# instadeepai/FrameDiPT

Measured on AMD Instinct MI355X. Metric: residue*diffusion-steps/sec, higher is better.
Workload: dtype fp16

## Files before the change

framedipt_amd/csrc/frames.hip:

```cpp
#include "common.hpp"
#include "kernels.hpp"
#include "philox.hpp"

#pragma clang fp contract(off)

__device__ __forceinline__ void d_quat_to_rot(const float* q, float* R) {
  const float a = q[0], b = q[1], c = q[2], d = q[3];
  R[0] = a * a + b * b - c * c - d * d; R[1] = 2 * b * c - 2 * a * d; R[2] = 2 * b * d + 2 * a * c;
  R[3] = 2 * b * c + 2 * a * d; R[4] = a * a - b * b + c * c - d * d; R[5] = 2 * c * d - 2 * a * b;
  R[6] = 2 * b * d - 2 * a * c; R[7] = 2 * c * d + 2 * a * b; R[8] = a * a - b * b - c * c + d * d;
}
__device__ __forceinline__ void d_quat_mul(const float* p, const float* q, float* o) {
  o[0] = p[0] * q[0] - p[1] * q[1] - p[2] * q[2] - p[3] * q[3];
  o[1] = p[0] * q[1] + p[1] * q[0] + p[2] * q[3] - p[3] * q[2];
  o[2] = p[0] * q[2] - p[1] * q[3] + p[2] * q[0] + p[3] * q[1];
  o[3] = p[0] * q[3] + p[1] * q[2] - p[2] * q[1] + p[3] * q[0];
}
__device__ __forceinline__ void d_quat_mul_vec(const float* q, const float* v, float* o) {
  o[0] = -q[1] * v[0] - q[2] * v[1] - q[3] * v[2];
  o[1] = q[0] * v[0] + q[2] * v[2] - q[3] * v[1];
  o[2] = q[0] * v[1] - q[1] * v[2] + q[3] * v[0];
  o[3] = q[0] * v[2] + q[1] * v[1] - q[2] * v[0];
}
__device__ __forceinline__ void d_invert_quat(const float* q, float* o) {
// ... 71 lines not shown
  for (int i = 0; i < 3; ++i)
    for (int j = 0; j < 3; ++j) Ro[i * 3 + j] = R1[i * 3] * R2[j] + R1[i * 3 + 1] * R2[3 + j] + R1[i * 3 + 2] * R2[6 + j];
  float tmp[3];
  d_rot_vec(R1, t2, tmp);
  to[0] = tmp[0] + t1[0]; to[1] = tmp[1] + t1[1]; to[2] = tmp[2] + t1[2];
}

__device__ __forceinline__ void d_backbone_residue(long r, const float* Rb, const float* tbv, const float* __restrict__ psi,
                                                   const int32_t* __restrict__ aatype, const BackboneTables* __restrict__ tb,
                                                   float* __restrict__ atom37, float* __restrict__ atom14) {
  int aa = aatype ? aatype[r] : 0;
  if (aa == 20) aa = 0;
  const float s = psi[r * 2], co = psi[r * 2 + 1];
  float FR[8][9], FT[8][3];
  for (int g = 0; g < 8; ++g) {
    const float* d44 = tb->default_frames + (aa * 8 + g) * 16;
    float Rd[9], td[3], Ra[9];
    for (int i = 0; i < 3; ++i) {
      for (int j = 0; j < 3; ++j) Rd[i * 3 + j] = d44[i * 4 + j];
      td[i] = d44[i * 4 + 3];
    }
    const float a0 = g == 0 ? 0.f : s, a1 = g == 0 ? 1.f : co;
    Ra[0] = 1; Ra[1] = 0; Ra[2] = 0; Ra[3] = 0; Ra[4] = a1; Ra[5] = -a0; Ra[6] = 0; Ra[7] = a0; Ra[8] = a1;
    const float z3[3] = {0.f, 0.f, 0.f};
    d_compose(Rd, td, Ra, z3, FR[g], FT[g]);
  }
  for (int g = 5; g < 8; ++g) {
    float Rn[9], tn[3];
    d_compose(FR[g - 1], FT[g - 1], FR[g], FT[g], Rn, tn);
    for (int c = 0; c < 9; ++c) FR[g][c] = Rn[c];
    for (int c = 0; c < 3; ++c) FT[g][c] = tn[c];
  }
  float pos[14][3];
  for (int at = 0; at < 14; ++at) {
    const int g = tb->group_idx[aa * 14 + at];
    float Rg[9], tg[3], p[3];
    d_compose(Rb, tbv, FR[g], FT[g], Rg, tg);
    d_rot_vec(Rg, tb->ideal_pos + (aa * 14 + at) * 3, p);
    const float mk = tb->atom_mask[aa * 14 + at];
    for (int c = 0; c < 3; ++c) pos[at][c] = (p[c] + tg[c]) * mk;
  }
  if (atom14)
    for (int at = 0; at < 14; ++at)
      for (int c = 0; c < 3; ++c) fd_st(atom14 + (r * 14 + at) * 3 + c, pos[at][c]);
  if (atom37) {
    for (int c = 0; c < 37 * 3; ++c) atom37[r * 111 + c] = 0.f;
    const int map[5] = {0, 1, 2, 4, 3};
    for (int at = 0; at < 5; ++at)
      for (int c = 0; c < 3; ++c) fd_st(atom37 + r * 111 + at * 3 + c, pos[map[at]][c]);
  }
}

__device__ __forceinline__ void d_backbone_atom(int at, int aa, float s, float co, const float* Rb, const float* tbv,
                                                const BackboneTables* __restrict__ tb, float* p3) {
  const int g = tb->group_idx[aa * 14 + at];
  auto frame = [&](int gg, float* R, float* T) {
    const float* d44 = tb->default_frames + (aa * 8 + gg) * 16;
    float Rd[9], td[3], Ra[9];
    for (int i = 0; i < 3; ++i) {
      for (int j = 0; j < 3; ++j) Rd[i * 3 + j] = d44[i * 4 + j];
      td[i] = d44[i * 4 + 3];
    }
    const float a0 = gg == 0 ? 0.f : s, a1 = gg == 0 ? 1.f : co;
    Ra[0] = 1; Ra[1] = 0; Ra[2] = 0; Ra[3] = 0; Ra[4] = a1; Ra[5] = -a0; Ra[6] = 0; Ra[7] = a0; Ra[8] = a1;
    const float z3[3] = {0.f, 0.f, 0.f};
    d_compose(Rd, td, Ra, z3, R, T);
  };
  float FRg[9], FTg[3];
  frame(g < 5 ? g : 4, FRg, FTg);
  for (int gg = 5; gg <= g; ++gg) {
    float Rc[9], Tc[3], Rn[9], Tn[3];
    frame(gg, Rc, Tc);
    d_compose(FRg, FTg, Rc, Tc, Rn, Tn);
    for (int c = 0; c < 9; ++c) FRg[c] = Rn[c];
    for (int c = 0; c < 3; ++c) FTg[c] = Tn[c];
  }
  float Rg[9], tg[3], p[3];
  d_compose(Rb, tbv, FRg, FTg, Rg, tg);
  d_rot_vec(Rg, tb->ideal_pos + (aa * 14 + at) * 3, p);
  const float mk = tb->atom_mask[aa * 14 + at];
  for (int c = 0; c < 3; ++c) p3[c] = (p[c] + tg[c]) * mk;
}

struct ReverseArgs {
  int B, N;
  const float* rigids_t;
  const double* rot_score;
  const float* trans_score;
  const float* diffuse_mask;
  const double *z_rot, *z_trans;
  double t, dt, noise_scale;
  int center, diffuse_rot, diffuse_trans;
  double so3_min_sigma, so3_max_sigma, r3_min_b, r3_max_b, cs;
  float* rigids_out;
  float* out_rot;
  int rpb;
  const float* psi;
  const int32_t* aatype;
  const BackboneTables* tables;
  float* atom37;
  const float* pred_rigids;
  const float* traj_fixed;
  float* trans_traj;
  int32_t* cursor = nullptr;
  const double* t_table = nullptr;
};

struct NoiseKeys { const uint64_t* keys; int step; };
template <bool GEN, typename... G>
__global__ __launch_bounds__(FD_THREADS) void reverse_step_kernel(ReverseArgs a, G... gs) {
  static_assert(sizeof...(G) == (GEN ? 1 : 0), "noise keys ride along with GEN only");
  __shared__ double red[4][FD_THREADS / 64];
  __shared__ double com[4];
  const int b = blockIdx.y, tid = threadIdx.x, lane = tid & 63, wave = tid >> 6;
  const int N = a.N;
  uint64_t key = 0;
  int step = 0;
  if constexpr (GEN) {
    const NoiseKeys g = (gs, ...);
    key = g.keys[b];
    step = a.cursor ? a.cursor[0] : g.step;
  }
  if (a.cursor) {
    const long s = a.cursor[0], R = (long)a.B * N;
    a.rigids_t += s * R * 7;
    a.rigids_out += (s + 1) * R * 7;
    if (!GEN) {
      a.z_rot += s * R * 3;
      a.z_trans += s * R * 3;
    }
    a.t = a.t_table[s];
    if (a.atom37) a.atom37 += s * R * 111;
    if (a.trans_traj) a.trans_traj += s * R * 3;
  }
  const double emax = exp(a.so3_max_sigma), emin = exp(a.so3_min_sigma);
  const double sig = log(a.t * emax + (1 - a.t) * emin);
  const double g_rot = sqrt(2 * (emax - emin) * sig / exp(sig));
  const double bt = a.r3_min_b + a.t * (a.r3_max_b - a.r3_min_b);
  const double g_tr = sqrt(bt);
  const double sdt = sqrt(a.dt);
  double sx = 0, sy = 0, sz = 0, sm = 0;
  for (int i = tid; i < N; i += FD_THREADS) {
    const long r = (long)b * N + i;
    const double m = a.diffuse_mask ? (double)a.diffuse_mask[r] : 1.0;
    double x1[3], zt[3] = {0.0, 0.0, 0.0};
    if (GEN && a.diffuse_trans) fd_noise3(key, (uint32_t)i, (uint32_t)step, FD_NOISE_REV_TRANS, zt);
    for (int c = 0; c < 3; ++c) {
      const double x = (double)a.rigids_t[r * 7 + 4 + c] * a.cs;
      const double f = -0.5 * bt * x;
      const double z = a.noise_scale * (GEN ? zt[c] : a.z_trans[r * 3 + c]);
      double pert = (f - g_tr * g_tr * (double)a.trans_score[r * 3 + c]) * a.dt + g_tr * sdt * z;
      pert *= m;
      x1[c] = x - pert;
    }
    sx += x1[0]; sy += x1[1]; sz += x1[2]; sm += m;
  }
  sx = wave_sum_d(sx); sy = wave_sum_d(sy); sz = wave_sum_d(sz); sm = wave_sum_d(sm);
  if (lane == 0) { red[0][wave] = sx; red[1][wave] = sy; red[2][wave] = sz; red[3][wave] = sm; }
  __syncthreads();
  if (tid < 4) {
    double s = 0;
    for (int w = 0; w < FD_THREADS / 64; ++w) s += red[tid][w];
    com[tid] = s;
  }
  __syncthreads();
  const double cx = a.center ? com[0] / com[3] : 0.0, cy = a.center ? com[1] / com[3] : 0.0,
               cz = a.center ? com[2] / com[3] : 0.0;
  const int i_end = (int)(blockIdx.x + 1) * a.rpb < N ? (int)(blockIdx.x + 1) * a.rpb : N;
  for (int i = blockIdx.x * a.rpb + tid; i < i_end; i += FD_THREADS) {
    const long r = (long)b * N + i;
    const bool has_mask = a.diffuse_mask != nullptr;
    const double m = has_mask ? (double)a.diffuse_mask[r] : 1.0;
    double tr_out[3], zt[3] = {0.0, 0.0, 0.0}, zr[3] = {0.0, 0.0, 0.0};
    if (GEN && a.diffuse_trans) fd_noise3(key, (uint32_t)i, (uint32_t)step, FD_NOISE_REV_TRANS, zt);
    for (int c = 0; c < 3; ++c) {
      const double xt = (double)a.rigids_t[r * 7 + 4 + c];
      double x1 = xt;
      if (a.diffuse_trans) {
        const double x = xt * a.cs;
        const double f = -0.5 * bt * x;
        const double z = a.noise_scale * (GEN ? zt[c] : a.z_trans[r * 3 + c]);
        double pert = (f - g_tr * g_tr * (double)a.trans_score[r * 3 + c]) * a.dt + g_tr * sdt * z;
        pert *= m;
        x1 = x - pert;
        x1 -= (c == 0 ? cx : (c == 1 ? cy : cz));
        x1 = x1 / a.cs;
      }
      tr_out[c] = has_mask ? (m * x1 + (1 - m) * xt) : x1;
    }
    float R32[9];
    d_quat_to_rot(a.rigids_t + r * 7, R32);
    double Rt[9], Ro[9];
    for (int c = 0; c < 9; ++c) Rt[c] = (double)R32[c];
    double pert[3];
    if (GEN && a.diffuse_rot) fd_noise3(key, (uint32_t)i, (uint32_t)step, FD_NOISE_REV_ROT, zr);
    for (int c = 0; c < 3; ++c)
      pert[c] = g_rot * g_rot * a.rot_score[r * 3 + c] * a.dt + g_rot * sdt * (a.noise_scale * (GEN ? zr[c] : a.z_rot[r * 3 + c]));
    if (!has_mask || m == 1.0 || m == 0.0) {
      double q0[4];
      d_markley(Rt, q0);
      if (a.diffuse_rot && m != 0.0) {
        double Re[9], Rp[9], Rc[9], q1[4];
        d_quat_matrix(q0, Re);
        d_so3_exp(pert, Rp);
        for (int ii = 0; ii < 3; ++ii)
          for (int jj = 0; jj < 3; ++jj)
            Rc[ii * 3 + jj] = Re[ii * 3] * Rp[jj] + Re[ii * 3 + 1] * Rp[3 + jj] + Re[ii * 3 + 2] * Rp[6 + jj];
        d_markley(Rc, q1);
        d_quat_matrix(q1, Ro);
      } else {
        d_quat_matrix(q0, Ro);
      }
    } else {
    double rv[3];
    d_so3_log(Rt, rv);
    double rv1[3] = {rv[0], rv[1], rv[2]};
    if (a.diffuse_rot) {
      double Rp[9], Rc[9];
      double Re[9];
      d_so3_exp(rv, Re);
      d_so3_exp(pert, Rp);
      for (int ii = 0; ii < 3; ++ii)
        for (int jj = 0; jj < 3; ++jj)
          Rc[ii * 3 + jj] = Re[ii * 3] * Rp[jj] + Re[ii * 3 + 1] * Rp[3 + jj] + Re[ii * 3 + 2] * Rp[6 + jj];
      d_so3_log(Rc, rv1);
    }
    if (has_mask)
      for (int c = 0; c < 3; ++c) rv1[c] = m * rv1[c] + (1 - m) * rv[c];
    d_so3_exp(rv1, Ro);
    }
    float Rf[9];
    for (int c = 0; c < 9; ++c) Rf[c] = (float)Ro[c];
    if (a.out_rot)
      for (int c = 0; c < 9; ++c) fd_st(a.out_rot + r * 9 + c, Rf[c]);
    double Rd[9], q[4];
    for (int c = 0; c < 9; ++c) Rd[c] = (double)Rf[c];
    d_markley(Rd, q);
    if (q[3] < 0) { q[0] = -q[0]; q[1] = -q[1]; q[2] = -q[2]; q[3] = -q[3]; }
    float* o = a.rigids_out + r * 7;
    fd_st(o, (float)q[3]); fd_st(o + 1, (float)q[0]); fd_st(o + 2, (float)q[1]); fd_st(o + 3, (float)q[2]);
    fd_st(o + 4, (float)tr_out[0]); fd_st(o + 5, (float)tr_out[1]); fd_st(o + 6, (float)tr_out[2]);
    if (a.atom37) {
      const float tf[3] = {o[4], o[5], o[6]};
      d_backbone_residue(r, Rf, tf, a.psi, a.aatype, a.tables, a.atom37, nullptr);
    }
    if (a.trans_traj) {
      const float dm = a.diffuse_mask ? a.diffuse_mask[r] : 1.f, fm = a.traj_fixed[r];
      for (int c = 0; c < 3; ++c) fd_st(a.trans_traj + r * 3 + c, dm * a.pred_rigids[r * 7 + 4 + c] + fm * o[4 + c]);
    }
  }
  if (a.cursor) {
    __syncthreads();
// ... 520 lines not shown
}

#define FD_EW_EXPORT(name, X, Y, O, O2)                                                        \
  if (n <= 0) return FDIPT_OK;                                                                 \
  if (!(X) || !(O)) return FDIPT_EINVAL;                                                       \
  hipLaunchKernelGGL(name##_k, dim3(cdiv(n, 256)), dim3(256), 0, (hipStream_t)s, n, X, Y, O, O2); \
  FD_CHECK_LAUNCH();                                                                           \
  return FDIPT_OK;

extern "C" {
int fdipt_quat_to_rot(int n, const float* quat, float* rot, fdipt_stream_t s) { FD_EW_EXPORT(quat_to_rot, quat, nullptr, rot, nullptr) }
int fdipt_rot_to_quat(int n, const float* rot, float* quat, fdipt_stream_t s) { FD_EW_EXPORT(rot_to_quat, rot, nullptr, quat, nullptr) }
int fdipt_quat_multiply(int n, const float* q1, const float* q2, float* out, fdipt_stream_t s) { FD_EW_EXPORT(quat_multiply, q1, q2, out, nullptr) }
int fdipt_quat_multiply_by_vec(int n, const float* q, const float* v, float* out, fdipt_stream_t s) { FD_EW_EXPORT(quat_multiply_by_vec, q, v, out, nullptr) }
int fdipt_invert_quat(int n, const float* q, float* out, fdipt_stream_t s) { FD_EW_EXPORT(invert_quat, q, nullptr, out, nullptr) }
int fdipt_rigid_apply(int n, const float* t7, const float* pts, float* out, fdipt_stream_t s) { FD_EW_EXPORT(rigid_apply, t7, pts, out, nullptr) }
int fdipt_rigid_invert_apply(int n, const float* t7, const float* pts, float* out, fdipt_stream_t s) { FD_EW_EXPORT(rigid_invert_apply, t7, pts, out, nullptr) }
int fdipt_rigid_compose(int n, const float* a, const float* b, float* out_rot, float* out_trans, fdipt_stream_t s) { FD_EW_EXPORT(rigid_compose, a, b, out_rot, out_trans) }
int fdipt_rigid_invert(int n, const float* t7, float* out_rot, float* out_trans, fdipt_stream_t s) { FD_EW_EXPORT(rigid_invert, t7, nullptr, out_rot, out_trans) }
int fdipt_quat_to_rotvec(int n, const float* q, float* rotvec, fdipt_stream_t s) { FD_EW_EXPORT(quat_to_rotvec, q, nullptr, rotvec, nullptr) }

int fdipt_rigid_compose_q_update(int n, const float* t7, const float* upd6, const float* mask, float* out_t7,
                                 fdipt_stream_t s) {
  if (n <= 0) return FDIPT_OK;
  if (!t7 || !upd6 || !out_t7) return FDIPT_EINVAL;
  hipLaunchKernelGGL(cqu_t7_k, dim3(cdiv(n, 256)), dim3(256), 0, (hipStream_t)s, n, t7, upd6, mask, out_t7);
  FD_CHECK_LAUNCH();
  return FDIPT_OK;
}
int fdipt_rigid_from_3_points(int n, const float* p_neg_x_axis, const float* origin, const float* p_xy_plane, float eps, float* rot,
                              fdipt_stream_t s) {
  if (n <= 0) return FDIPT_OK;
  if (!p_neg_x_axis || !origin || !p_xy_plane || !rot) return FDIPT_EINVAL;
  hipLaunchKernelGGL(from_3_points_k, dim3(cdiv(n, 256)), dim3(256), 0, (hipStream_t)s, n, p_neg_x_axis, origin, p_xy_plane, eps, rot);
  FD_CHECK_LAUNCH();
  return FDIPT_OK;
}
int fdipt_so3_exp_geomstats(int n, const double* rotvec, double* rot, fdipt_stream_t s) {
  if (n <= 0) return FDIPT_OK;
  if (!rotvec || !rot) return FDIPT_EINVAL;
  hipLaunchKernelGGL(gs_exp_k, dim3(cdiv(n, 256)), dim3(256), 0, (hipStream_t)s, n, rotvec, rot);
  FD_CHECK_LAUNCH();
  return FDIPT_OK;
}
int fdipt_so3_log_geomstats(int n, const double* rot, double* rotvec, fdipt_stream_t s) {
  if (n <= 0) return FDIPT_OK;
  if (!rotvec || !rot) return FDIPT_EINVAL;
  hipLaunchKernelGGL(gs_log_k, dim3(cdiv(n, 256)), dim3(256), 0, (hipStream_t)s, n, rot, rotvec);
  FD_CHECK_LAUNCH();
  return FDIPT_OK;
}
int fdipt_so3_omega(int n, const double* rot, double eps, double* angle, fdipt_stream_t s) {
  if (n <= 0) return FDIPT_OK;
  if (!angle || !rot) return FDIPT_EINVAL;
  hipLaunchKernelGGL(gs_omega_k, dim3(cdiv(n, 256)), dim3(256), 0, (hipStream_t)s, n, rot, eps, angle);
  FD_CHECK_LAUNCH();
  return FDIPT_OK;
}
int fdipt_so3_exp(int n, const double* rotvec, double* rot, fdipt_stream_t s) {
  if (n <= 0) return FDIPT_OK;
  if (!rotvec || !rot) return FDIPT_EINVAL;
  hipLaunchKernelGGL(so3_exp_k, dim3(cdiv(n, 256)), dim3(256), 0, (hipStream_t)s, n, rotvec, rot);
  FD_CHECK_LAUNCH();
  return FDIPT_OK;
}
int fdipt_so3_log(int n, const double* rot, double* rotvec, fdipt_stream_t s) {
  if (n <= 0) return FDIPT_OK;
  if (!rot || !rotvec) return FDIPT_EINVAL;
  hipLaunchKernelGGL(so3_log_k, dim3(cdiv(n, 256)), dim3(256), 0, (hipStream_t)s, n, rot, rotvec);
  FD_CHECK_LAUNCH();
  return FDIPT_OK;
}

int fdipt_se3_reverse_step_atoms(int B, int N, const float* rigids_t, const double* rot_score, const float* trans_score,
                                 const float* diffuse_mask, const double* z_rot, const double* z_trans, double t, double dt,
                                 double noise_scale, int center, int diffuse_rot, int diffuse_trans, double so3_min_sigma,
                                 double so3_max_sigma, double r3_min_b, double r3_max_b, double coordinate_scaling,
                                 float* rigids_out, float* out_rot, const float* psi, const int32_t* aatype,
                                 const void* tables, float* atom37, fdipt_stream_t stream) {
  if (B <= 0 || N <= 0) return FDIPT_OK;
  if (!rigids_t || !rot_score || !trans_score || !z_rot || !z_trans || !rigids_out || !(t >= 0 && t <= 1))
    return FDIPT_EINVAL;
  if (atom37 && (!psi || !tables || rigids_out == rigids_t)) return FDIPT_EINVAL;
  const int rpb = rigids_out == rigids_t ? N : 64;
  ReverseArgs a = {B, N, rigids_t, rot_score, trans_score, diffuse_mask, z_rot, z_trans, t, dt, noise_scale, center,
                   diffuse_rot, diffuse_trans, so3_min_sigma, so3_max_sigma, r3_min_b, r3_max_b, coordinate_scaling,
                   rigids_out, out_rot, rpb, psi, aatype, (const BackboneTables*)tables, atom37, nullptr, nullptr, nullptr};
  hipLaunchKernelGGL(reverse_step_kernel<false>, dim3(cdiv(N, rpb), B), dim3(FD_THREADS), 0, (hipStream_t)stream, a);
  FD_CHECK_LAUNCH();
  return FDIPT_OK;
}
int fdipt_se3_reverse_step_traj(int B, int N, const float* rigids_t, const double* rot_score, const float* trans_score,
                                const float* diffuse_mask, const double* z_rot, const double* z_trans, double t, double dt,
                                double noise_scale, int center, int diffuse_rot, int diffuse_trans, double so3_min_sigma,
                                double so3_max_sigma, double r3_min_b, double r3_max_b, double coordinate_scaling,
                                float* rigids_out, float* out_rot, const float* psi, const int32_t* aatype,
                                const void* tables, float* atom37, const float* pred_rigids, const float* traj_fixed_mask,
                                float* trans_traj, fdipt_stream_t stream) {
  if (B <= 0 || N <= 0) return FDIPT_OK;
  if (!rigids_t || !rot_score || !trans_score || !z_rot || !z_trans || !rigids_out || !(t >= 0 && t <= 1))
    return FDIPT_EINVAL;
  if (atom37 && (!psi || !tables || rigids_out == rigids_t)) return FDIPT_EINVAL;
  if (trans_traj && (!pred_rigids || !traj_fixed_mask)) return FDIPT_EINVAL;
  const int rpb = rigids_out == rigids_t ? N : 64;
  ReverseArgs a = {B, N, rigids_t, rot_score, trans_score, diffuse_mask, z_rot, z_trans, t, dt, noise_scale, center,
                   diffuse_rot, diffuse_trans, so3_min_sigma, so3_max_sigma, r3_min_b, r3_max_b, coordinate_scaling,
                   rigids_out, out_rot, rpb, psi, aatype, (const BackboneTables*)tables, atom37, pred_rigids, traj_fixed_mask, trans_traj};
  hipLaunchKernelGGL(reverse_step_kernel<false>, dim3(cdiv(N, rpb), B), dim3(FD_THREADS), 0, (hipStream_t)stream, a);
  FD_CHECK_LAUNCH();
  return FDIPT_OK;
}
int fdipt_se3_reverse_step_indexed(const FdiptReverseIndexed* x, fdipt_stream_t stream) {
  if (!x) return FDIPT_EINVAL;
  if (x->B <= 0 || x->N <= 0) return FDIPT_OK;
  if (!x->rigid_traj || !x->rot_score || !x->trans_score || !x->z_rot || !x->z_trans || !x->t_table || !x->step_cursor) return FDIPT_EINVAL;
  if (x->prot_traj && (!x->psi || !x->bb_tables)) return FDIPT_EINVAL;
  if (x->trans_traj && (!x->pred_rigids || !x->traj_fixed_mask)) return FDIPT_EINVAL;
  ReverseArgs a = {x->B, x->N, x->rigid_traj, x->rot_score, x->trans_score, x->diffuse_mask, x->z_rot, x->z_trans, 0.0, x->dt,
                   x->noise_scale, x->center, x->diffuse_rot, x->diffuse_trans, x->so3_min_sigma, x->so3_max_sigma, x->r3_min_b,
                   x->r3_max_b, x->coordinate_scaling, x->rigid_traj, nullptr, 64, x->psi, x->aatype,
                   (const BackboneTables*)x->bb_tables, x->prot_traj, x->pred_rigids, x->traj_fixed_mask, x->trans_traj,
                   x->step_cursor, x->t_table};
  hipLaunchKernelGGL(reverse_step_kernel<false>, dim3(cdiv(x->N, 64), x->B), dim3(FD_THREADS), 0, (hipStream_t)stream, a);
  FD_CHECK_LAUNCH();
  return FDIPT_OK;
}
int fdipt_se3_reverse_step_traj_gen(int B, int N, const float* rigids_t, const double* rot_score, const float* trans_score,
                                    const float* diffuse_mask, const uint64_t* noise_keys, int step, double t, double dt,
                                    double noise_scale, int center, int diffuse_rot, int diffuse_trans, double so3_min_sigma,
                                    double so3_max_sigma, double r3_min_b, double r3_max_b, double coordinate_scaling,
                                    float* rigids_out, float* out_rot, const float* psi, const int32_t* aatype,
                                    const void* tables, float* atom37, const float* pred_rigids, const float* traj_fixed_mask,
                                    float* trans_traj, fdipt_stream_t stream) {
  if (B <= 0 || N <= 0) return FDIPT_OK;
  if (!rigids_t || !rot_score || !trans_score || !noise_keys || step < 0 || !rigids_out || !(t >= 0 && t <= 1))
    return FDIPT_EINVAL;
  if (atom37 && (!psi || !tables || rigids_out == rigids_t)) return FDIPT_EINVAL;
  if (trans_traj && (!pred_rigids || !traj_fixed_mask)) return FDIPT_EINVAL;
  const int rpb = rigids_out == rigids_t ? N : 64;
  ReverseArgs a = {B, N, rigids_t, rot_score, trans_score, diffuse_mask, nullptr, nullptr, t, dt, noise_scale, center,
                   diffuse_rot, diffuse_trans, so3_min_sigma, so3_max_sigma, r3_min_b, r3_max_b, coordinate_scaling,
                   rigids_out, out_rot, rpb, psi, aatype, (const BackboneTables*)tables, atom37, pred_rigids, traj_fixed_mask, trans_traj};
  hipLaunchKernelGGL((reverse_step_kernel<true, NoiseKeys>), dim3(cdiv(N, rpb), B), dim3(FD_THREADS), 0, (hipStream_t)stream, a, NoiseKeys{noise_keys, step});
  FD_CHECK_LAUNCH();
  return FDIPT_OK;
}
int fdipt_se3_reverse_step_indexed_gen(const FdiptReverseIndexed* x, const uint64_t* noise_keys, fdipt_stream_t stream) {
  if (!x) return FDIPT_EINVAL;
  if (x->B <= 0 || x->N <= 0) return FDIPT_OK;
  if (!x->rigid_traj || !x->rot_score || !x->trans_score || x->z_rot || x->z_trans || !noise_keys || !x->t_table || !x->step_cursor)
    return FDIPT_EINVAL;
  if (x->prot_traj && (!x->psi || !x->bb_tables)) return FDIPT_EINVAL;
  if (x->trans_traj && (!x->pred_rigids || !x->traj_fixed_mask)) return FDIPT_EINVAL;
  ReverseArgs a = {x->B, x->N, x->rigid_traj, x->rot_score, x->trans_score, x->diffuse_mask, nullptr, nullptr, 0.0, x->dt,
                   x->noise_scale, x->center, x->diffuse_rot, x->diffuse_trans, x->so3_min_sigma, x->so3_max_sigma, x->r3_min_b,
                   x->r3_max_b, x->coordinate_scaling, x->rigid_traj, nullptr, 64, x->psi, x->aatype,
                   (const BackboneTables*)x->bb_tables, x->prot_traj, x->pred_rigids, x->traj_fixed_mask, x->trans_traj,
                   x->step_cursor, x->t_table};
  hipLaunchKernelGGL((reverse_step_kernel<true, NoiseKeys>), dim3(cdiv(x->N, 64), x->B), dim3(FD_THREADS), 0, (hipStream_t)stream, a, NoiseKeys{noise_keys, 0});
  FD_CHECK_LAUNCH();
  return FDIPT_OK;
}
int fdipt_noise_fill(int B, int N, const uint64_t* noise_keys, int purpose, int k_begin, int n_steps, double* out, fdipt_stream_t stream) {
  if (B <= 0 || N <= 0 || n_steps <= 0) return FDIPT_OK;
  if (!noise_keys || !out || purpose < 0 || purpose >= (int)FD_NOISE_PURPOSES || k_begin < 0) return FDIPT_EINVAL;
  const long n = (long)n_steps * B * N;
  hipLaunchKernelGGL(noise_fill_kernel, dim3(cdiv(n, FD_THREADS)), dim3(FD_THREADS), 0, (hipStream_t)stream, B, N, noise_keys,
                     (uint32_t)purpose, k_begin, n, out);
  FD_CHECK_LAUNCH();
  return FDIPT_OK;
}
int fdipt_se3_reverse_step(int B, int N, const float* rigids_t, const double* rot_score, const float* trans_score,
                           const float* diffuse_mask, const double* z_rot, const double* z_trans, double t, double dt,
                           double noise_scale, int center, int diffuse_rot, int diffuse_trans, double so3_min_sigma,
                           double so3_max_sigma, double r3_min_b, double r3_max_b, double coordinate_scaling,
                           float* rigids_out, float* out_rot, fdipt_stream_t stream) {
  return fdipt_se3_reverse_step_atoms(B, N, rigids_t, rot_score, trans_score, diffuse_mask, z_rot, z_trans, t, dt, noise_scale,
                                      center, diffuse_rot, diffuse_trans, so3_min_sigma, so3_max_sigma, r3_min_b, r3_max_b,
                                      coordinate_scaling, rigids_out, out_rot, nullptr, nullptr, nullptr, nullptr, stream);
}

int fdipt_igso3_rot_score(int B, int N, const float* quats_t, const float* quats_0, const double* sigma,
                          const float* res_mask, double* score, fdipt_stream_t s) {
  if (B <= 0 || N <= 0) return FDIPT_OK;
  if (!quats_t || !quats_0 || !sigma || !score) return FDIPT_EINVAL;
  return fd_rot_score(B, N, quats_t, 4, quats_0, 4, sigma, res_mask, score, (hipStream_t)s);
}
int fdipt_igso3_rot_score_cached(int B, int N, const float* quats_t, const float* quats_0, const double* score_table,
                                 const double* omega_edges, int n_omega, const float* res_mask, double* score, fdipt_stream_t s) {
  if (B <= 0 || N <= 0) return FDIPT_OK;
  if (!quats_t || !quats_0 || !score_table || !omega_edges || n_omega < 2 || !score) return FDIPT_EINVAL;
  ScoreTail x = {};
  x.score_table = score_table; x.omega_edges = omega_edges; x.n_omega = n_omega;
  hipLaunchKernelGGL(rot_score_kernel, dim3(cdiv((long)B * N, FD_THREADS / RS_LANES)), dim3(FD_THREADS), 0, (hipStream_t)s, B, N, quats_t, 4,
                     quats_0, 4, score_table, res_mask, score, x);
  FD_CHECK_LAUNCH();
  return FDIPT_OK;
}
int fdipt_r3_trans_score(int B, int N, const float* trans_t, const float* trans_0, const float* t, float min_b,
                         float max_b, float coordinate_scaling, const float* res_mask, float* score, fdipt_stream_t s) {
  if (B <= 0 || N <= 0) return FDIPT_OK;
  if (!trans_t || !trans_0 || !t || !score) return FDIPT_EINVAL;
  return fd_trans_score(B, N, trans_t, 3, trans_0, 3, t, min_b, max_b, coordinate_scaling, res_mask, score, (hipStream_t)s);
}
int fdipt_backbone_atoms(int n, const float* t7, const float* rot, const float* trans, const float* psi,
                         const int32_t* aatype, const void* tables, float* atom37, float* atom14, fdipt_stream_t s) {
  if (n <= 0) return FDIPT_OK;
  if ((!t7 && !(rot && trans)) || !psi || !tables) return FDIPT_EINVAL;
  return fd_backbone(n, t7, rot, trans, 3, psi, aatype, tables, atom37, atom14, (hipStream_t)s);
}
int fdipt_backbone_atoms_indexed(int n, const float* t7, const float* psi, const int32_t* aatype, const void* tables,
                                 float* atom37_rows, const int32_t* step_cursor, fdipt_stream_t s) {
  if (n <= 0) return FDIPT_OK;
  if (!t7 || !psi || !tables || !atom37_rows || !step_cursor) return FDIPT_EINVAL;
  return fd_backbone(n, t7, nullptr, nullptr, 3, psi, aatype, tables, atom37_rows, nullptr, (hipStream_t)s, step_cursor);
}
}

struct SdeConsts { double so3_min_sigma, so3_max_sigma, r3_min_b, r3_max_b, cs; };
__device__ __forceinline__ double d_g_rot(const SdeConsts& k, double t) {
  const double emax = exp(k.so3_max_sigma), emin = exp(k.so3_min_sigma);
  const double sig = log(t * emax + (1 - t) * emin);
  return sqrt(2 * (emax - emin) * sig / exp(sig));
}
__device__ __forceinline__ double d_b_t(const SdeConsts& k, double t) { return k.r3_min_b + t * (k.r3_max_b - k.r3_min_b); }
__device__ __forceinline__ void d_matmul3(const double* A, const double* B, double* C) {
  for (int i = 0; i < 3; ++i)
    for (int j = 0; j < 3; ++j) C[i * 3 + j] = A[i * 3] * B[j] + A[i * 3 + 1] * B[3 + j] + A[i * 3 + 2] * B[6 + j];
}
__device__ __forceinline__ void d_compose_rotvec(const double* r1, const double* r2, double* out) {
  double R1[9], R2[9], Rc[9];
  d_so3_exp(r1, R1);
  d_so3_exp(r2, R2);
  d_matmul3(R1, R2, Rc);
  d_so3_log(Rc, out);
}
__device__ __forceinline__ void d_align_rotvec(const double* in, const double* target, double* out) {
  const double ang = sqrt(in[0] * in[0] + in[1] * in[1] + in[2] * in[2]);
  const double tn = sqrt(target[0] * target[0] + target[1] * target[1] + target[2] * target[2]);
  const double ax[3] = {in[0] / ang, in[1] / ang, in[2] / ang};
  const double dot = (target[0] / tn) * ax[0] + (target[1] / tn) * ax[1] + (target[2] / tn) * ax[2];
  const double sign = dot > 0 ? 1.0 : (dot < 0 ? -1.0 : dot);
// ... 200 lines not shown
```

framedipt_amd/csrc/model.hip:

```cpp
#include <math.h>
#include <string.h>

#include <vector>

#include "common.hpp"
#include "kernels.hpp"

struct LinW { long w, b; int out, in; };
struct LNW { long g, b; int d; };
#define FD_MAX_BLOCKS 8
#define FD_MAX_TL 4
struct TfLayer { LinW inp, outp, l1, l2; LNW n1, n2; };
struct BlockW {
  long head_w;
  LinW q, kv, qp, kvp, lb, dz, out, rbf;
  LNW ipa_ln;
  LinW skip;
  TfLayer tf[FD_MAX_TL];
  LinW post, t1, t2, t3;
  LNW tln;
  LinW bb;
  LinW et_init, et1, et2, etf;
  LNW et_ln;
};
// ... 975 lines not shown
    const DBlock& db = L.blk[b];
    const int cs = d->c_s, dt = iv.d_t;
    if (p.post == POST_CHAIN) {
      ChainArgs c;
      c.M = R; c.in = x; c.ld_in = dt; c.w[0] = D + db.ch.post; c.b[0] = P + k.post.b; c.residual = F(w.tf_in); c.ld_res = dt;
      c.out = F(w.h_a); c.ld_out = cs;
      if (p.rbk) c.warm = warm_of(b, WARM_TRANSITION32);
      RC(fd_chain(FD_CHAIN_POST, c, st));
    } else if (p.post == POST_GEMM) RC(lin(k.post, x, dt, F(w.tf_in), dt, nullptr, 0, F(w.h_a), cs));
    if (p.transition == NF_GEMM) {
      RC(lin(k.t1, F(w.h_a), cs, nullptr, 0, nullptr, 1, F(w.h_b), cs));
      RC(lin(k.t2, F(w.h_b), cs, nullptr, 0, nullptr, 1, F(w.ipa_out), cs));
      RC(lin(k.t3, F(w.ipa_out), cs, F(w.h_a), cs, nullptr, 0, F(w.h_b), cs));
      RC(fd_layernorm(R, cs, F(w.h_b), cs, nullptr, 0, P + k.tln.g, P + k.tln.b, a->res_mask, F(w.node), cs, st));
      RC(lin32(k.bb, F(w.node), cs, F(w.upd), 8));
      RC(inner(b, 3, F(w.upd), 8, 6));
      return fd_compose_q_update(R, F(w.quat), F(w.trans), F(w.upd), 8, F(w.dmask), st);
    }
    const bool r16 = p.transition == NF_ROWS16;
    RowBlockArgs r;
    r.M = R; r.in = F(w.h_a); r.ld_in = cs;
    r.w0 = D + (r16 ? db.lo.tr16[0][0] : db.ch.t1); r.w1 = D + (r16 ? db.lo.tr16[1][0] : db.ch.t2); r.w2 = D + (r16 ? db.lo.tr16[2][0] : db.ch.t3);
    if (p.split) { r.w0l = D + (r16 ? db.lo.tr16[0][1] : db.lo.t1); r.w1l = D + (r16 ? db.lo.tr16[1][1] : db.lo.t2); r.w2l = D + (r16 ? db.lo.tr16[2][1] : db.lo.t3); }
    r.b0 = P + k.t1.b; r.b1 = P + k.t2.b; r.b2 = P + k.t3.b; r.residual = F(w.h_a); r.ld_res = cs; r.gamma = P + k.tln.g; r.beta = P + k.tln.b;
    r.rowmask_post = a->res_mask; r.out = F(w.node); r.ld_out = cs; r.bb_w = P + k.bb.w; r.bb_b = P + k.bb.b;
    r.upd_mask = F(w.dmask); r.quat = F(w.quat); r.trans = F(w.trans);
    if (b < d->num_blocks - 1 && p.et_widths) r.warm = warm_of(b, WARM_ET_ROWS);
    else if (b == d->num_blocks - 1) r.warm = warm_of(b, WARM_TORSION);
    if (fold_et_rows(b)) {
      r.we0 = D + db.lo.ei16[0]; r.we0l = D + db.lo.ei16[1]; r.we1 = D + db.lo.r416[0]; r.we1l = D + db.lo.r416[1];
      r.be0 = P + k.et_init.b; r.be1 = (const float*)(D + db.ch.r4b);
      r.img_a = W + w.a1img; r.img_b = W + w.b1img; r.img_B = B; r.img_N = N;
      r.warm = warm_of(b, WARM_ET_FOLDED);
    }
    if (r16) return fd_transition16(r, st);
    return fd_rowblock(p.split ? FD_RB_TRANSITION_BB_SPLIT : FD_RB_TRANSITION_BB, r, st);
  }
  int edge_transition_stage(int b, const float* node) const {
    const BlockW& k = iv.blk[b];
    const DBlock& db = L.blk[b];
    const int cs = d->c_s, cz = d->c_z;
    RowBlockArgs r;
    r.M = R; r.in = node; r.ld_in = cs; r.w0 = D + db.ch.et_init; r.b0 = P + k.et_init.b;
    if (p.et == ET_ET4 && !fold_et_rows(b)) {
      r.w1 = D + db.ch.r4w; r.b1 = (const float*)(D + db.ch.r4b); r.out = F(w.r4); r.ld_out = 1024;
      r.img_a = W + w.a1img; r.img_b = W + w.b1img; r.img_B = B; r.img_N = N;
      if (p.et_rows == ETR_ROWS) {
        RC(fd_rowblock(FD_RB_ET4_ROWS, r, st));
        RC(fd_et4_row_images(F(w.r4), B, N, W + w.a1img, W + w.b1img, st));
      } else {
        if (p.split) { r.w0l = D + db.lo.et_init; r.w1l = D + db.lo.r4w; }
        RC(fd_rowblock(FD_RB_ET4_IMAGES, r, st));
      }
    } else if (p.et == ET_ET3) {
      r.w1 = D + db.ch.a1af; r.b1 = (const float*)(D + db.ch.b1f); r.out = F(w.a1); r.ld_out = iv.hid; r.out2 = F(w.af); r.ld_out2 = cz;
      r.split = iv.hid; r.hid_h16 = (unsigned short*)(W + w.e_bf);
      RC(fd_rowblock(FD_RB_ET_ROWS, r, st));
    } else if (p.et == ET_CHAIN) {
      ChainArgs c;
      c.M = R; c.in = node; c.ld_in = cs; c.w[0] = D + db.ch.et_init; c.b[0] = P + k.et_init.b; c.out_h16 = (unsigned short*)(W + w.e_bf);
      c.out = F(w.e); c.ld_out = iv.cb;
      RC(fd_chain(FD_CHAIN_ETINIT, c, st));
    } else if (p.et == ET_GEMM) {
      RC(lin(k.et_init, node, cs, nullptr, 0, nullptr, 0, F(w.e), iv.cb));
      if (p.bf) RC(fd_f32_to_half((long)R * iv.cb, F(w.e), (half_t*)(W + w.e_bf), st));
    }
    float* tr_ptr = a->trace_edge ? a->trace_edge + (size_t)(b + 1) * NN * cz : nullptr;
    if (a->ev_start && a->ev_start[b]) hipEventRecord((hipEvent_t)a->ev_start[b], st);
    if (p.et == ET_ET4 || p.et == ET_ET3) {
      ET2Args t2;
      t2.B = B; t2.N = N; t2.z_in = (const half_t*)(W + w.z); t2.z_out = (half_t*)(W + w.z); t2.e = F(w.e);
      t2.e_h16 = (const half_t*)(W + w.e_bf);
      t2.a1 = F(w.a1); t2.af = F(w.af); t2.stream = D + (p.et == ET_ET3 ? db.et3 : p.x ? db.et4x : db.et4); t2.b2 = P + k.et2.b; t2.gamma = P + k.et_ln.g;
      t2.beta = P + k.et_ln.b; t2.res_mask = a->res_mask; t2.trace = tr_ptr;
      const DBlock& next = L.blk[b + 1];
      t2.wb_img = p.et_bias ? D + (p.et == ET_ET4 ? next.wb_img4 : next.wb_img3) : nullptr;
      t2.a1_img = W + w.a1img; t2.b1_img = W + w.b1img;
      t2.bb = (const float*)(D + next.bb); t2.bias_out = F(w.bias); t2.H = d->no_heads; t2.reserve_cus = a->reserve_cus;
      if (p.pz) {
        t2.bdz = P + iv.blk[b + 1].dz.b; t2.pz_out = (half_t*)(W + w.pz);
        if (b + 1 == d->num_blocks - 1 && !tr_ptr) t2.z_out = nullptr;
      }
      t2.clock = a->clock_out;
      if (p.et == ET_ET4) RC(fd_edge_transition4(t2, st, p.x));
      else RC(fd_edge_transition3(t2, st));
    } else {
      EdgeTransArgs ta;
      ta.B = B; ta.N = N; ta.z_in = W + w.z; ta.z_out = W + w.z; ta.e = F(w.e);
      ta.w1 = WM(k.et1); ta.w2 = WM(k.et2); ta.wf = WM(k.etf); ta.b1 = P + k.et1.b; ta.b2 = P + k.et2.b; ta.bf = P + k.etf.b;
      ta.gamma = P + k.et_ln.g; ta.beta = P + k.et_ln.b; ta.res_mask = a->res_mask; ta.trace = tr_ptr; ta.clock = a->clock_out;
      RC(fd_edge_transition(op_precision(d), cz, iv.cb, ta, st));
    }
    if (a->ev_stop && a->ev_stop[b]) hipEventRecord((hipEvent_t)a->ev_stop[b], st);
    return FDIPT_OK;
  }
  int heads_stage(const float* node) const {
    const int cs = d->c_s;
    if (p.torsion == NF_GEMM) {
      RC(lin(iv.tor1, node, cs, nullptr, 0, nullptr, 1, F(w.h_a), cs));
      RC(lin(iv.tor2, F(w.h_a), cs, node, cs, nullptr, 0, F(w.h_b), cs));
    } else {
      const bool r16 = p.torsion == NF_ROWS16;
      RowBlockArgs r;
      r.M = R; r.in = node; r.ld_in = cs; r.w0 = D + (r16 ? L.tor16[0][0] : L.ch_tor1); r.w1 = D + (r16 ? L.tor16[1][0] : L.ch_tor2);
      if (p.split) { r.w0l = D + (r16 ? L.tor16[0][1] : L.lo_tor1); r.w1l = D + (r16 ? L.tor16[1][1] : L.lo_tor2); }
      r.b0 = P + iv.tor1.b; r.b1 = P + iv.tor2.b; r.residual = node; r.ld_res = cs; r.out = F(w.h_b); r.ld_out = cs;
      if (r16) RC(fd_torsion16(r, st));
      else RC(fd_rowblock(p.split ? FD_RB_TORSION_SPLIT : FD_RB_TORSION, r, st));
    }
    if (!p.torf_fused) RC(lin32(iv.torf, F(w.h_b), cs, F(w.psi_un), 8));
    const bool atoms = a->atom37 || a->atom14;
    if (atoms && !a->bb_tables) return FDIPT_EINVAL;
    const bool bb_fold = atoms && p.bb_fold;
    RC(fd_score_tail(B, N, a->rigids_t, F(w.quat), F(w.trans), d->coordinate_scaling, F(w.psi_un), 8, a->gt_psi, a->fixed_mask,
                     a->res_mask, a->so3_sigma, a->t, d->r3_min_b, d->r3_max_b, a->rigids, a->psi, a->rot_score, a->trans_score,
                     a->ca_out, p.torf_fused ? F(w.h_b) : nullptr, cs, cs, P + iv.torf.w, P + iv.torf.b, a->so3_score_table,
                     a->so3_omega_edges, a->so3_num_omega, a->aatype, bb_fold ? a->bb_tables : nullptr, bb_fold ? a->atom37 : nullptr,
                     bb_fold ? a->atom14 : nullptr, a->step_cursor, st));
    if (atoms && !bb_fold)
      RC(fd_backbone(R, a->rigids, nullptr, nullptr, 0, a->psi, a->aatype, a->bb_tables, a->atom37, a->atom14, st, a->step_cursor));
    return FDIPT_OK;
  }
};

static int forward_impl(const FdiptDims* d, const float* P, const void* derived, const void* setup,
                        const FdiptForwardArgs* a, void* workspace, size_t workspace_bytes, fdipt_stream_t stream, const OpSel& op) {
  if (!dims_ok(d) || !P || !derived || !a || !workspace) return FDIPT_EINVAL;
  if (a->B <= 0 || a->N <= 0 || !a->res_mask) return FDIPT_EINVAL;
  if (op.kind == OP_ALL || op.kind == OP_EMBED) {
    if (!setup || !a->fixed_mask || (!a->sc_ca_t && d->num_bins > 0) || !a->seq_idx || !a->idx_emb || !a->t_emb) return FDIPT_EINVAL;
    if (d->use_aatype && (!a->aatype || !a->t_emb_eps)) return FDIPT_EINVAL;
  }
  if (op.kind == OP_ALL && (!a->rigids_t || !a->gt_psi || !a->t || !a->so3_sigma || !a->psi || !a->rot_score || !a->trans_score ||
                            !a->rigids))
    return FDIPT_EINVAL;
  if ((op.kind == OP_POINTS || op.kind == OP_IPA) && !a->rigids_t) return FDIPT_EINVAL;
  if (op.kind != OP_ALL && op.kind != OP_EMBED && (op.block < 0 || op.block >= d->num_blocks - (op.kind == OP_ET ? 1 : 0))) return FDIPT_EINVAL;
  Inventory iv;
  DLayout L;
  WS w;
  build_inventory(d, iv);
  blob_walk(d, iv, L);
  const int B = a->B, N = a->N, R = B * N;
  build_ws(d, iv, L, B, N, w);
  if (workspace_bytes < w.total) return FDIPT_ESIZE;
  if ((long)B * N * N > 2000000000L / 1) return FDIPT_ESIZE;
  const ForwardPlan p = plan_forward(d, iv, L, B, N, op.kind);
  if (p.refused) return FDIPT_EINVAL;
  const Fwd f = {d, iv, L, w, p, P, (const char*)derived, (char*)workspace, setup, a, (hipStream_t)stream, B, N, R, (N + 31) / 32 * 32, (size_t)R * N};
  if (a->trace_inner && (p.rbk || p.outproj != OUT_GEMM)) return FDIPT_EINVAL;
  const size_t node_bytes = (size_t)R * d->c_s * 4, z_bytes = f.NN * d->c_z * L.esz;
  if (op.kind == OP_ALL || op.kind == OP_EMBED) RC(f.embed_stage());
  if (op.kind == OP_EMBED) {
    if (op.node_out) RC(f.d2d(op.node_out, f.F(w.node0), node_bytes));
    if (op.z_out) RC(f.d2d(op.z_out, f.W + w.z, z_bytes));
    return FDIPT_OK;
  }
  if (a->trace_node && op.kind == OP_ALL) RC(f.d2d(a->trace_node, f.F(w.node0), node_bytes));
  if (!p.feats_fused && a->rigids_t)
    RC(fd_split_rigids(R, a->rigids_t, d->coordinate_scaling, a->res_mask, a->fixed_mask ? a->fixed_mask : a->res_mask, f.F(w.quat),
                       f.F(w.trans), f.F(w.dmask), a->step_cursor, f.st));
  if (op.kind != OP_ALL) {
    if (!op.node_in) return FDIPT_EINVAL;
    RC(f.d2d(f.F(w.node), op.node_in, node_bytes));
    if (op.kind != OP_POINTS) {
      if (!op.z_in) return FDIPT_EINVAL;
// ... 108 lines not shown
```

Baseline: 1.158 million.

## Widen reverse-step blocks to 512 threads and shrink residues per block

The reverse diffusion step kernel now launches with 512 threads instead of FD_THREADS. Each block still recomputes the full center-of-mass sum, but the upper half of the threads now stage their partial sums in shared memory so that only the lower four waves do the wave reductions. Residues per block drop from 64 to 16, which creates more blocks and spreads the per-residue frame and atom work across more CUs. The cost is that the redundant center-of-mass pass is repeated in more blocks and needs extra barriers. A validation check is also added in the edge-transition path.

```diff
diff --git a/framedipt_amd/csrc/frames.hip b/framedipt_amd/csrc/frames.hip
--- a/framedipt_amd/csrc/frames.hip
+++ b/framedipt_amd/csrc/frames.hip
@@ -177,6 +177,8 @@
   for (int c = 0; c < 3; ++c) p3[c] = (p[c] + tg[c]) * mk;
 }
 
+#define RS_THREADS 512
+#define RS_RPB 16
 struct ReverseArgs {
   int B, N;
   const float* rigids_t;
@@ -203,10 +205,11 @@
 
 struct NoiseKeys { const uint64_t* keys; int step; };
 template <bool GEN, typename... G>
-__global__ __launch_bounds__(FD_THREADS) void reverse_step_kernel(ReverseArgs a, G... gs) {
+__global__ __launch_bounds__(RS_THREADS) void reverse_step_kernel(ReverseArgs a, G... gs) {
   static_assert(sizeof...(G) == (GEN ? 1 : 0), "noise keys ride along with GEN only");
-  __shared__ double red[4][FD_THREADS / 64];
+  __shared__ double red[4][4];
   __shared__ double com[4];
+  __shared__ double hi[4][RS_THREADS / 2];
   const int b = blockIdx.y, tid = threadIdx.x, lane = tid & 63, wave = tid >> 6;
   const int N = a.N;
   uint64_t key = 0;
@@ -235,34 +238,48 @@
   const double g_tr = sqrt(bt);
   const double sdt = sqrt(a.dt);
   double sx = 0, sy = 0, sz = 0, sm = 0;
-  for (int i = tid; i < N; i += FD_THREADS) {
-    const long r = (long)b * N + i;
-    const double m = a.diffuse_mask ? (double)a.diffuse_mask[r] : 1.0;
-    double x1[3], zt[3] = {0.0, 0.0, 0.0};
-    if (GEN && a.diffuse_trans) fd_noise3(key, (uint32_t)i, (uint32_t)step, FD_NOISE_REV_TRANS, zt);
-    for (int c = 0; c < 3; ++c) {
-      const double x = (double)a.rigids_t[r * 7 + 4 + c] * a.cs;
-      const double f = -0.5 * bt * x;
-      const double z = a.noise_scale * (GEN ? zt[c] : a.z_trans[r * 3 + c]);
-      double pert = (f - g_tr * g_tr * (double)a.trans_score[r * 3 + c]) * a.dt + g_tr * sdt * z;
-      pert *= m;
-      x1[c] = x - pert;
-    }
-    sx += x1[0]; sy += x1[1]; sz += x1[2]; sm += m;
-  }
-  sx = wave_sum_d(sx); sy = wave_sum_d(sy); sz = wave_sum_d(sz); sm = wave_sum_d(sm);
-  if (lane == 0) { red[0][wave] = sx; red[1][wave] = sy; red[2][wave] = sz; red[3][wave] = sm; }
+  const int t = tid & (RS_THREADS / 2 - 1);
+  const bool upper = tid >= RS_THREADS / 2;
+  for (int i0 = 0; i0 < N; i0 += RS_THREADS) {
+    const int i = i0 + tid;
+    double x1[3] = {0.0, 0.0, 0.0}, m = 0.0;
+    if (i < N) {
+      const long r = (long)b * N + i;
+      m = a.diffuse_mask ? (double)a.diffuse_mask[r] : 1.0;
+      double zt[3] = {0.0, 0.0, 0.0};
+      if (GEN && a.diffuse_trans) fd_noise3(key, (uint32_t)i, (uint32_t)step, FD_NOISE_REV_TRANS, zt);
+      for (int c = 0; c < 3; ++c) {
+        const double x = (double)a.rigids_t[r * 7 + 4 + c] * a.cs;
+        const double f = -0.5 * bt * x;
+        const double z = a.noise_scale * (GEN ? zt[c] : a.z_trans[r * 3 + c]);
+        double pert = (f - g_tr * g_tr * (double)a.trans_score[r * 3 + c]) * a.dt + g_tr * sdt * z;
+        pert *= m;
+        x1[c] = x - pert;
+      }
+    }
+    if (i0 > 0) __syncthreads();
+    if (upper) { hi[0][t] = x1[0]; hi[1][t] = x1[1]; hi[2][t] = x1[2]; hi[3][t] = m; }
+    __syncthreads();
+    if (!upper) {
+      if (i < N) { sx += x1[0]; sy += x1[1]; sz += x1[2]; sm += m; }
+      if (i + RS_THREADS / 2 < N) { sx += hi[0][t]; sy += hi[1][t]; sz += hi[2][t]; sm += hi[3][t]; }
+    }
+  }
+  if (!upper) {
+    sx = wave_sum_d(sx); sy = wave_sum_d(sy); sz = wave_sum_d(sz); sm = wave_sum_d(sm);
+    if (lane == 0) { red[0][wave] = sx; red[1][wave] = sy; red[2][wave] = sz; red[3][wave] = sm; }
+  }
   __syncthreads();
   if (tid < 4) {
     double s = 0;
-    for (int w = 0; w < FD_THREADS / 64; ++w) s += red[tid][w];
+    for (int w = 0; w < 4; ++w) s += red[tid][w];
     com[tid] = s;
   }
   __syncthreads();
   const double cx = a.center ? com[0] / com[3] : 0.0, cy = a.center ? com[1] / com[3] : 0.0,
                cz = a.center ? com[2] / com[3] : 0.0;
   const int i_end = (int)(blockIdx.x + 1) * a.rpb < N ? (int)(blockIdx.x + 1) * a.rpb : N;
-  for (int i = blockIdx.x * a.rpb + tid; i < i_end; i += FD_THREADS) {
+  for (int i = blockIdx.x * a.rpb + tid; i < i_end; i += RS_THREADS) {
     const long r = (long)b * N + i;
     const bool has_mask = a.diffuse_mask != nullptr;
     const double m = has_mask ? (double)a.diffuse_mask[r] : 1.0;
@@ -949,11 +966,11 @@
   if (!rigids_t || !rot_score || !trans_score || !z_rot || !z_trans || !rigids_out || !(t >= 0 && t <= 1))
     return FDIPT_EINVAL;
   if (atom37 && (!psi || !tables || rigids_out == rigids_t)) return FDIPT_EINVAL;
-  const int rpb = rigids_out == rigids_t ? N : 64;
+  const int rpb = rigids_out == rigids_t ? N : RS_RPB;
   ReverseArgs a = {B, N, rigids_t, rot_score, trans_score, diffuse_mask, z_rot, z_trans, t, dt, noise_scale, center,
                    diffuse_rot, diffuse_trans, so3_min_sigma, so3_max_sigma, r3_min_b, r3_max_b, coordinate_scaling,
                    rigids_out, out_rot, rpb, psi, aatype, (const BackboneTables*)tables, atom37, nullptr, nullptr, nullptr};
-  hipLaunchKernelGGL(reverse_step_kernel<false>, dim3(cdiv(N, rpb), B), dim3(FD_THREADS), 0, (hipStream_t)stream, a);
+  hipLaunchKernelGGL(reverse_step_kernel<false>, dim3(cdiv(N, rpb), B), dim3(RS_THREADS), 0, (hipStream_t)stream, a);
   FD_CHECK_LAUNCH();
   return FDIPT_OK;
 }
@@ -969,11 +986,11 @@
     return FDIPT_EINVAL;
   if (atom37 && (!psi || !tables || rigids_out == rigids_t)) return FDIPT_EINVAL;
   if (trans_traj && (!pred_rigids || !traj_fixed_mask)) return FDIPT_EINVAL;
-  const int rpb = rigids_out == rigids_t ? N : 64;
+  const int rpb = rigids_out == rigids_t ? N : RS_RPB;
   ReverseArgs a = {B, N, rigids_t, rot_score, trans_score, diffuse_mask, z_rot, z_trans, t, dt, noise_scale, center,
                    diffuse_rot, diffuse_trans, so3_min_sigma, so3_max_sigma, r3_min_b, r3_max_b, coordinate_scaling,
                    rigids_out, out_rot, rpb, psi, aatype, (const BackboneTables*)tables, atom37, pred_rigids, traj_fixed_mask, trans_traj};
-  hipLaunchKernelGGL(reverse_step_kernel<false>, dim3(cdiv(N, rpb), B), dim3(FD_THREADS), 0, (hipStream_t)stream, a);
+  hipLaunchKernelGGL(reverse_step_kernel<false>, dim3(cdiv(N, rpb), B), dim3(RS_THREADS), 0, (hipStream_t)stream, a);
   FD_CHECK_LAUNCH();
   return FDIPT_OK;
 }
@@ -985,10 +1002,10 @@
   if (x->trans_traj && (!x->pred_rigids || !x->traj_fixed_mask)) return FDIPT_EINVAL;
   ReverseArgs a = {x->B, x->N, x->rigid_traj, x->rot_score, x->trans_score, x->diffuse_mask, x->z_rot, x->z_trans, 0.0, x->dt,
                    x->noise_scale, x->center, x->diffuse_rot, x->diffuse_trans, x->so3_min_sigma, x->so3_max_sigma, x->r3_min_b,
-                   x->r3_max_b, x->coordinate_scaling, x->rigid_traj, nullptr, 64, x->psi, x->aatype,
+                   x->r3_max_b, x->coordinate_scaling, x->rigid_traj, nullptr, RS_RPB, x->psi, x->aatype,
                    (const BackboneTables*)x->bb_tables, x->prot_traj, x->pred_rigids, x->traj_fixed_mask, x->trans_traj,
                    x->step_cursor, x->t_table};
-  hipLaunchKernelGGL(reverse_step_kernel<false>, dim3(cdiv(x->N, 64), x->B), dim3(FD_THREADS), 0, (hipStream_t)stream, a);
+  hipLaunchKernelGGL(reverse_step_kernel<false>, dim3(cdiv(x->N, RS_RPB), x->B), dim3(RS_THREADS), 0, (hipStream_t)stream, a);
   FD_CHECK_LAUNCH();
   return FDIPT_OK;
 }
@@ -1004,11 +1021,11 @@
     return FDIPT_EINVAL;
   if (atom37 && (!psi || !tables || rigids_out == rigids_t)) return FDIPT_EINVAL;
   if (trans_traj && (!pred_rigids || !traj_fixed_mask)) return FDIPT_EINVAL;
-  const int rpb = rigids_out == rigids_t ? N : 64;
+  const int rpb = rigids_out == rigids_t ? N : RS_RPB;
   ReverseArgs a = {B, N, rigids_t, rot_score, trans_score, diffuse_mask, nullptr, nullptr, t, dt, noise_scale, center,
                    diffuse_rot, diffuse_trans, so3_min_sigma, so3_max_sigma, r3_min_b, r3_max_b, coordinate_scaling,
                    rigids_out, out_rot, rpb, psi, aatype, (const BackboneTables*)tables, atom37, pred_rigids, traj_fixed_mask, trans_traj};
-  hipLaunchKernelGGL((reverse_step_kernel<true, NoiseKeys>), dim3(cdiv(N, rpb), B), dim3(FD_THREADS), 0, (hipStream_t)stream, a, NoiseKeys{noise_keys, step});
+  hipLaunchKernelGGL((reverse_step_kernel<true, NoiseKeys>), dim3(cdiv(N, rpb), B), dim3(RS_THREADS), 0, (hipStream_t)stream, a, NoiseKeys{noise_keys, step});
   FD_CHECK_LAUNCH();
   return FDIPT_OK;
 }
@@ -1021,10 +1038,10 @@
   if (x->trans_traj && (!x->pred_rigids || !x->traj_fixed_mask)) return FDIPT_EINVAL;
   ReverseArgs a = {x->B, x->N, x->rigid_traj, x->rot_score, x->trans_score, x->diffuse_mask, nullptr, nullptr, 0.0, x->dt,
                    x->noise_scale, x->center, x->diffuse_rot, x->diffuse_trans, x->so3_min_sigma, x->so3_max_sigma, x->r3_min_b,
-                   x->r3_max_b, x->coordinate_scaling, x->rigid_traj, nullptr, 64, x->psi, x->aatype,
+                   x->r3_max_b, x->coordinate_scaling, x->rigid_traj, nullptr, RS_RPB, x->psi, x->aatype,
                    (const BackboneTables*)x->bb_tables, x->prot_traj, x->pred_rigids, x->traj_fixed_mask, x->trans_traj,
                    x->step_cursor, x->t_table};
-  hipLaunchKernelGGL((reverse_step_kernel<true, NoiseKeys>), dim3(cdiv(x->N, 64), x->B), dim3(FD_THREADS), 0, (hipStream_t)stream, a, NoiseKeys{noise_keys, 0});
+  hipLaunchKernelGGL((reverse_step_kernel<true, NoiseKeys>), dim3(cdiv(x->N, RS_RPB), x->B), dim3(RS_THREADS), 0, (hipStream_t)stream, a, NoiseKeys{noise_keys, 0});
   FD_CHECK_LAUNCH();
   return FDIPT_OK;
 }
diff --git a/framedipt_amd/csrc/model.hip b/framedipt_amd/csrc/model.hip
--- a/framedipt_amd/csrc/model.hip
+++ b/framedipt_amd/csrc/model.hip
@@ -1081,6 +1081,7 @@
         if (b + 1 == d->num_blocks - 1 && !tr_ptr) t2.z_out = nullptr;
       }
       t2.clock = a->clock_out;
+      if (!t2.z_out && !t2.pz_out) return FDIPT_EINVAL;
       if (p.et == ET_ET4) RC(fd_edge_transition4(t2, st, p.x));
       else RC(fd_edge_transition3(t2, st));
     } else {
```

After: 1.156 million. No clear change (-0.2%).
